# ruppelb/Large-Scale-ViT-SLAM

Hardware: AMD Instinct MI355X
Metric: chunks/sec (16-frame 518x518) + ViT MFMA util% (higher is better)
Workload: dtype bf16; 1 GPU; VGGT aggregator forward (DINOv2-L/14-reg + 24x frame/global AA blocks), 1 chunk of 16 frames 518x518, layers 4/11/17/23 emitted; frames=16, parallelism=replicas x1

## Files before the change

### include/vggt_mi355x.h

```cpp
#ifndef VGGT_MI355X_H
#define VGGT_MI355X_H

#include <stddef.h>
#include <stdint.h>

#ifdef __cplusplus
extern "C" {
#endif

#define VGGT_OK 0
#define VGGT_ERR_SHAPE (-1)
#define VGGT_ERR_ALIGN (-2)
#define VGGT_ERR_HIP (-3)
#define VGGT_ERR_UNSUPPORTED (-4)

#define VGGT_DTYPE_F32 0
#define VGGT_DTYPE_BF16 1

#define VGGT_EPI_BF16 0
#define VGGT_EPI_GELU_BF16 1
#define VGGT_EPI_RESID_F32 2
#define VGGT_EPI_F32 3

#define VGGT_ROPE_NONE 0
#define VGGT_ROPE_2D 1
#define VGGT_ROPE_1D 2

const char* vggt_version(void);

#define VGGT_TUNE_GEMM_TILE 1
#define VGGT_TUNE_ATTN_WAVES 2
#define VGGT_TUNE_ATTN_VARIANT 3
#define VGGT_TUNE_CONV_PF2 4
#define VGGT_TUNE_ATTN16 5
#define VGGT_TUNE_LINEAR_ONE_LAUNCH 6
#define VGGT_TUNE_LINEAR_SPLIT_K 7
#define VGGT_TUNE_LINEAR_WK 8
#define VGGT_TUNE_GEMM_BALANCE 10
#define VGGT_TUNE_ATTN_TAIL_SPLIT 11
int vggt_tune(int knob, int value);

#define VGGT_STREAM_SHORT_WORKGROUPS 1
int vggt_set_stream_config(void* stream, int cus, int flags);

int vggt_gemm_bf16(const void* A, int64_t lda, const void* W, int64_t ldw, const float* bias, int M, int N, int K,
                   int epi, void* out, int64_t ldo, const float* gamma, float* out2, int64_t ldo2, void* stream);

int vggt_gemm_bf16_gelu_pre(const void* A, int64_t lda, const void* W, int64_t ldw, const float* bias, int M, int N,
                            int K, void* out, int64_t ldo, void* pre, int64_t ldp, void* stream);

int vggt_gemm_qkv(const void* A, int64_t lda, const void* W, int64_t ldw, const float* bias, int M, int H, int D, int K,
                  void* out, int64_t ldo, const float* qw, const float* qb, const float* kw, const float* kb, float eps,
                  int rope_mode, const int32_t* pos, int period, const float* cos_tab, const float* sin_tab,
                  int tab_len, void* stream);

int vggt_gemm_headnorm(const void* A, int64_t lda, const void* W, int64_t ldw, const float* bias, int M, int N, int H,
                       int D, int K, void* out, int64_t ldo, const float* nw, const float* nb, float eps, int rope_mode,
                       const int32_t* pos, int period, const float* cos_tab, const float* sin_tab, int tab_len,
                       void* stream);

#define VGGT_GEMM_ENTRY_BF16 0
#define VGGT_GEMM_ENTRY_GELU_PRE 1
#define VGGT_GEMM_ENTRY_QKV 2
#define VGGT_GEMM_ENTRY_HEADNORM 3
#define VGGT_GEMM_FAMILY_128 0
#define VGGT_GEMM_FAMILY_RING 1
#define VGGT_GEMM_FAMILY_TWO 2
#define VGGT_GEMM_FAMILY_PP 3
#define VGGT_GEMM_FAMILY_PPP 4
typedef struct {
  int family;
  int bm, bn;
  int epi;
  int fk;
  int grid, lds;
  int sched;
  int split_rows;
  int rc;
  int dev_cus;
} vggt_gemm_form_t;
int vggt_gemm_form(int entry, int epi, int has_out2, int M, int N, int K, int H, int D, int rope_mode, int period,
                   int tab_len, int64_t lda, int64_t ldw, int64_t ldo, int64_t ldo2, int stream_cus, int stream_flags,
                   int force, vggt_gemm_form_t* form);

int vggt_layernorm(const void* x, int in_dtype, int64_t ldx, const float* w, const float* b, float eps, int M, int C,
                   void* y, int out_dtype, int64_t ldy, void* stream);

int vggt_resid_add_layernorm(float* x, int64_t ldx, const void* y, int64_t ldy, const float* gamma, float* out2,
                             int64_t ldo2, const float* w, const float* b, float eps, int M, int C, void* xn,
                             int64_t ldn, void* stream);

int vggt_resid_add_layernorm_nostore(const float* x, int64_t ldx, const void* y, int64_t ldy, const float* gamma,
                                     const float* w, const float* b, float eps, int M, int C, void* xn, int64_t ldn,
                                     void* stream);
int vggt_resid_add2_layernorm(float* x, int64_t ldx, const void* y, int64_t ldy, const float* gamma, const void* y2,
                              int64_t ldy2, const float* gamma2, float* out2, int64_t ldo2, const float* w,
                              const float* b, float eps, int M, int C, void* xn, int64_t ldn, void* stream);

int vggt_headnorm_rope(void* buf, int64_t ld, int col_off, int M, int H, int D, const float* w, const float* b,
                       float eps, int rope_mode, const int32_t* pos, int period, const float* cos_tab,
                       const float* sin_tab, int tab_len, void* stream);

int vggt_qknorm_rope(void* qkv, int64_t ld, int M, int H, int D, const float* qw, const float* qb, const float* kw,
                     const float* kb, float eps, int rope_mode, const int32_t* pos, int period, const float* cos_tab,
                     const float* sin_tab, int tab_len, void* stream);

int vggt_qknorm_rope_out(const void* src, int64_t lds, void* dst, int64_t ldd, int M, int H, int D, const float* qw,
                         const float* qb, const float* kw, const float* kb, float eps, int rope_mode,
                         const int32_t* pos, int period, const float* cos_tab, const float* sin_tab, int tab_len,
                         void* stream);
int vggt_headnorm_rope_out(const void* src, int64_t lds, void* dst, int64_t ldd, int M, int H, int D, const float* w,
                           const float* b, float eps, int rope_mode, const int32_t* pos, int period,
                           const float* cos_tab, const float* sin_tab, int tab_len, void* stream);

int vggt_attention_fwd(const void* q, int64_t ldq, int64_t q_bstride, const void* k, int64_t ldk, int64_t k_bstride,
                       const void* v, int64_t ldv, int64_t v_bstride, void* o, int64_t ldo, int64_t o_bstride,
                       int batch, int heads, int nq, int nk, int D, float scale, void* stream);

int vggt_attention_fwd_ws(const void* q, int64_t ldq, int64_t q_bstride, const void* k, int64_t ldk,
                          int64_t k_bstride, const void* v, int64_t ldv, int64_t v_bstride, void* o, int64_t ldo,
                          int64_t o_bstride, int batch, int heads, int nq, int nk, int D, float scale, void* ws,
                          size_t ws_bytes, void* stream);
// ... 187 lines not shown
```

### large-scale-vit-slam_amd/aligned_vggt/_native.py

```python
from __future__ import annotations

import ctypes
import os
from typing import Optional

import torch

from .runtime import Workspace, scratch_table

_PKG_ROOT = os.path.dirname(os.path.dirname(os.path.abspath(__file__)))
LIB_PATH = os.environ.get("VGGT_MI355X_LIB", os.path.join(_PKG_ROOT, "lib", "libvggt_mi355x.so"))
HEADER_PATH = os.path.join(os.path.dirname(_PKG_ROOT), "include", "vggt_mi355x.h")

VGGT_OK, VGGT_ERR_SHAPE, VGGT_ERR_ALIGN, VGGT_ERR_HIP, VGGT_ERR_UNSUPPORTED = 0, -1, -2, -3, -4
DTYPE_F32, DTYPE_BF16 = 0, 1
EPI_BF16, EPI_GELU_BF16, EPI_RESID_F32, EPI_F32 = 0, 1, 2, 3
ROPE_NONE, ROPE_2D, ROPE_1D = 0, 1, 2

_ERR = {VGGT_ERR_SHAPE: "unsupported or inconsistent shape", VGGT_ERR_ALIGN: "misaligned pointer or leading dimension",
        VGGT_ERR_HIP: "HIP launch/runtime error", VGGT_ERR_UNSUPPORTED: "unsupported mode or dtype"}

_vp, _i, _i64, _f = ctypes.c_void_p, ctypes.c_int, ctypes.c_int64, ctypes.c_float
_SIGS = {
    "vggt_tune": [_i, _i],
# ... 52 lines not shown
    "vggt_upsample_bilinear_f32": [_vp, _i, _i, _i, _i, _vp, _i, _i, _vp, _vp],
    "vggt_dpt_activate": [_vp, _i64, _i64, _i, _i, _i, _vp, _vp, _vp, _vp],
    "vggt_irls_sim3": [_vp, _i64, _vp, _i64, _vp, _i64, _vp, _i64, _i, _i64, _f, _f, _i, _f, _vp, _vp, _vp, _vp,
                       ctypes.c_size_t, _vp],
    "vggt_sim3_points": [_vp, _i64, _i, _i64, _vp, _vp, _vp, _i64, _vp],
    "vggt_scale_f32": [_vp, _i64, _i, _i64, _vp, _vp],
    "vggt_pose_compose": [_vp, _vp, _vp, _vp, _i, _vp, _i, _i, _i, _i, _i, _vp, _vp, _vp],
    "vggt_attention_fwd_lse": [_vp, _i64, _i64, _vp, _i64, _i64, _vp, _i64, _i64, _vp, _i64, _i64, _vp, _i, _i, _i,
                               _i, _i, _f, _vp],
    "vggt_attention_bwd": [_vp, _i64, _i64, _vp, _i64, _i64, _vp, _i64, _vp, _vp, _i64, _i64, _vp, _vp, _vp, _i64,
                           _vp, _vp, _i64, _i, _i, _i, _i, _i, _f, _vp],
    "vggt_attention_small_bwd": [_vp, _i64, _i64, _vp, _i64, _i64, _vp, _i64, _vp, _i64, _i64, _vp, _i64, _i64, _vp,
                                 _vp, _i64, _i64, _i, _i, _i, _i, _i, _i, _f, _vp],
    "vggt_layernorm_bwd": [_vp, _i, _i64, _vp, _f, _vp, _i, _i64, _vp, _i, _i64, _i, _i, _i, _i, _i, _i, _i, _i, _vp,
                           _vp, _vp, ctypes.c_size_t, _vp],
    "vggt_headnorm_rope_bwd": [_vp, _i64, _vp, _i64, _i, _i, _i, _i, _i, _vp, _vp, _f, _i, _vp, _i, _vp, _vp, _i, _vp,
                               _vp, _vp, _vp, _vp, ctypes.c_size_t, _vp],
    "vggt_colsum": [_vp, _i, _i64, _i, _i, _vp, _i, _vp, ctypes.c_size_t, _vp],
    "vggt_layerscale_bwd": [_vp, _i64, _vp, _i, _i64, _vp, _vp, _i, _i64, _i, _i, _vp, _vp, _vp, ctypes.c_size_t,
                            _vp],
    "vggt_gelu_fwd": [_vp, _i, _i64, _vp, _i, _i64, _i, _i, _vp],
    "vggt_gelu_bwd": [_vp, _i, _i64, _vp, _i, _i64, _vp, _i, _i64, _i, _i, _vp, _vp, ctypes.c_size_t, _vp],
    "vggt_resid_scale_add": [_vp, _i64, _vp, _i, _i64, _vp, _i, _i, _vp],
    "vggt_gemm_bf16_gelu_pre": [_vp, _i64, _vp, _i64, _vp, _i, _i, _i, _vp, _i64, _vp, _i64, _vp],
    "vggt_resid_scale_add_from": [_vp, _i64, _vp, _i64, _vp, _i, _i64, _vp, _i, _i, _vp],
    "vggt_qknorm_rope_out": [_vp, _i64, _vp, _i64, _i, _i, _i, _vp, _vp, _vp, _vp, _f, _i, _vp, _i, _vp, _vp, _i, _vp],
    "vggt_headnorm_rope_out": [_vp, _i64, _vp, _i64, _i, _i, _i, _vp, _vp, _f, _i, _vp, _i, _vp, _vp, _i, _vp],
    "vggt_transpose_b16": [_vp, _i64, _i, _i, _vp, _i64, _i, _vp],
    "vggt_wgrad_f32": [_vp, _i64, _vp, _i64, _i, _i, _i, _vp, _i64, _i, _vp],
    "vggt_wgrad_bias_f32": [_vp, _i64, _vp, _i64, _i, _i, _i, _vp, _i64, _vp, _i, _vp],
    "vggt_wgrad_bf16": [_vp, _i64, _vp, _i64, _i, _i, _i, _vp, _i64, _i, _vp, ctypes.c_size_t, _vp],
    "vggt_batch_dot_f32": [_vp, _vp, _i64, _i, _i64, _vp, _vp, ctypes.c_size_t, _vp],
    "vggt_nn1": [_vp, _i64, _vp, _vp, _i64, _vp, _i, _i64, _i64, _i, _vp, _vp, _i, _vp, ctypes.c_size_t, _vp],
    "vggt_nn1_plan": [_i, _i64, _i64, _i],
    "vggt_nn1_pair_stats": [_vp, _i64, _vp, _vp, _i64, _vp, _vp, _i, _i64, _i64, _vp, _vp, ctypes.c_size_t, _vp],
}
_WS_FNS = {"vggt_colred_workspace_bytes": [_i, _i], "vggt_layernorm_bwd_workspace_bytes": [_i, _i],
           "vggt_headnorm_rope_bwd_workspace_bytes": [_i, _i], "vggt_batch_dot_workspace_bytes": [_i, _i64],
           "vggt_wgrad_bf16_workspace_bytes": [_i, _i, _i], "vggt_attention_ws_bytes": [_i, _i, _i, _i, _i, _vp],
           "vggt_nn1_workspace_bytes": [_i, _i64, _i64]}

_lib = None

EVENT_HOOK = None


def lib() -> ctypes.CDLL:
    global _lib
    if _lib is None:
        if not os.path.exists(LIB_PATH):
            raise RuntimeError(f"libvggt_mi355x.so not found at {LIB_PATH}: build it with "
                               f"`make -C large-scale-vit-slam_amd/csrc` (or __graft_entry__.build()); "
                               f"there is no CPU fallback for the HIP hot path")
        L = ctypes.CDLL(LIB_PATH)
        for name, argt in _SIGS.items():
            fn = getattr(L, name)
            fn.argtypes = argt
            fn.restype = ctypes.c_int
        L.vggt_version.restype = ctypes.c_char_p
        L.vggt_irls_workspace_bytes.argtypes = [_i]
        L.vggt_irls_workspace_bytes.restype = ctypes.c_size_t
        for name, argt in _WS_FNS.items():
            fn = getattr(L, name)
            fn.argtypes = argt
            fn.restype = ctypes.c_size_t
        _lib = L
    return _lib


def version() -> str:
    return lib().vggt_version().decode()


TUNE_GEMM_TILE = 1
TUNE_ATTN_WAVES = 2
TUNE_ATTN_VARIANT = 3
TUNE_CONV_PF2 = 4
TUNE_ATTN16 = 5
TUNE_LINEAR_ONE_LAUNCH = 6
TUNE_LINEAR_SPLIT_K = 7
TUNE_LINEAR_WK = 8
TUNE_GEMM_BALANCE = 10
TUNE_ATTN_TAIL_SPLIT = 11


def tune(knob: int, value: int) -> int:
    rc = lib().vggt_tune(knob, value)
    if rc == VGGT_ERR_UNSUPPORTED:
        raise ValueError(f"vggt_tune: unsupported knob/value ({knob}, {value})")
    return rc


STREAM_SHORT_WORKGROUPS = 1


def set_stream_config(stream: int, cus: int, flags: int = 0) -> int:
    rc = lib().vggt_set_stream_config(ctypes.c_void_p(stream), cus, flags)
    if rc < 0:
        raise ValueError(f"vggt_set_stream_config: rejected ({rc})")
    return rc


def mfma_probe(iters: int = 200_000, random: bool = True, seconds: float = 2.0, device=None) -> dict:
    import statistics
    device = torch.device(device or "cuda")
    ncu = torch.cuda.get_device_properties(device).multi_processor_count
    g = torch.Generator(device="cpu").manual_seed(0)
    n = ncu * 256 * 16
    ops = (torch.randn(n, generator=g) if random else torch.zeros(n)).to(torch.bfloat16).to(device)
    stamps = torch.zeros(ncu * 4, dtype=torch.int64, device=device)
    sink = torch.empty(ncu * 256, dtype=torch.float32, device=device)
    st = ctypes.c_void_p(torch.cuda.current_stream(device).cuda_stream)
    launch = lambda: _check(lib().vggt_mfma_probe(_p(stamps), _p(sink), _p(ops), ncu, iters, st),
                            "vggt_mfma_probe")
    import time
    t_end = time.perf_counter() + seconds
    while time.perf_counter() < t_end:
        launch()
        torch.cuda.synchronize(device)
    a = torch.cuda.Event(enable_timing=True)
    b = torch.cuda.Event(enable_timing=True)
    a.record()
    launch()
    b.record()
    b.synchronize()
    ms = a.elapsed_time(b)
    sp = stamps.view(ncu, 4).cpu().tolist()
    clocks = [(t1 - t0) / (r1 - r0) * 100e6 for t0, t1, r0, r1 in sp if r1 > r0]
    clk = statistics.median(clocks)
    flop = ncu * 4 * iters * 8 * 32768.0
    return {"tflops": round(flop / (ms * 1e-3) / 1e12, 1), "clock_ghz": round(clk / 1e9, 3),
            "flop_per_cycle_per_cu": round(flop / ncu / (ms * 1e-3 * clk), 1), "ms": round(ms, 3), "cus": ncu,
            "operands": "random bf16" if random else "zeros"}


def _check(rc: int, name: str) -> None:
    if rc != VGGT_OK:
        raise RuntimeError(f"{name}: {_ERR.get(rc, 'error')} (code {rc})")


def _dev(t: torch.Tensor, name: str) -> None:
    if t.device.type != "cuda":
        raise RuntimeError(f"{name}: tensor on {t.device}; the MI355X hot path runs on HIP devices only")


def _p(t: Optional[torch.Tensor]):
    return None if t is None else ctypes.c_void_p(t.data_ptr())


def _stream() -> ctypes.c_void_p:
    return ctypes.c_void_p(torch.cuda.current_stream().cuda_stream)


def _ld(t: torch.Tensor) -> int:
    if t.dim() != 2 or t.stride(1) != 1:
        raise RuntimeError("expected a 2-D row-major (unit inner stride) view")
    return t.stride(0)


def gemm_bf16(a: torch.Tensor, w: torch.Tensor, bias: torch.Tensor, out: torch.Tensor, epi: int,
              gamma: Optional[torch.Tensor] = None, out2: Optional[torch.Tensor] = None) -> torch.Tensor:
    _dev(a, "gemm_bf16")
    M, K = a.shape
    N = w.shape[0]
    assert a.dtype == torch.bfloat16 and w.dtype == torch.bfloat16 and w.shape[1] == K
    assert out.shape[0] == M and out.shape[1] == N
# ... 813 lines not shown
```

### large-scale-vit-slam_amd/csrc/attention.hip

```cpp
#include <math.h>
#include <string.h>

#include <algorithm>
#include <mutex>
#include <type_traits>
#include <vector>

#include "common.h"
#include "tune.h"

namespace {

typedef __attribute__((ext_vector_type(4))) short s16x4;
typedef __attribute__((ext_vector_type(8))) short s16x8;
typedef int int32x4 __attribute__((ext_vector_type(4)));

constexpr int BKV = 64;
constexpr float THR = 8.0f;

struct AttnArgs {
  const bf16_t* q;
  const bf16_t* k;
  const bf16_t* v;
  bf16_t* o;
  int64_t ldq, ldk, ldv, ldo;
  int64_t qbs, kbs, vbs, obs;
  int batch, heads, nq, nk;
  float c;
  float* lse;
  int n_full, parts, part_tiles;
  float* ws;
};

constexpr int SPLIT_BQ = 256;
constexpr int SPLIT_SLAB = SPLIT_BQ * 64 + 2 * SPLIT_BQ;

__device__ __forceinline__ void dma16(int32x4 rsrc, uint32_t voff, uint32_t lds) {
  uint32_t keep;
  asm volatile("s_mov_b32 %0, m0\n\ts_mov_b32 m0, %3\n\ts_nop 0\n\tbuffer_load_dwordx4 %1, %2, 0 offen lds\n\t"
               "s_mov_b32 m0, %0"
               : "=&s"(keep)
               : "v"(voff), "s"(rsrc), "s"(lds)
               : "memory");
}

__device__ __forceinline__ int32x4 make_rsrc(const void* base, uint32_t nbytes) {
  const uint64_t b = (uint64_t)base;
  int32x4 r;
  r[0] = __builtin_amdgcn_readfirstlane((uint32_t)b);
  r[1] = __builtin_amdgcn_readfirstlane((uint32_t)(b >> 32)) & 0xffff;
  r[2] = __builtin_amdgcn_readfirstlane(nbytes);
  r[3] = 0x00020000;
  return r;
}

template <int D>
__device__ __forceinline__ int k_swz(int row, int chunk) {
  if constexpr (D == 64) return chunk ^ ((row >> 1) & 7);
  else return chunk ^ (row & 15);
}
template <int D>
__device__ __forceinline__ int v_swz(int row, int chunk) {
  if constexpr (D == 64) return chunk ^ (((row >> 1) & 1) << 2);
  else return chunk ^ ((row & 3) << 2);
}

constexpr int V_HOIST_K = 1;
constexpr int V_MAX4 = 2;
constexpr int V_SUM4 = 4;
constexpr int V_MFMA_SUM = 8;
constexpr int V_PIPE_QK = 16;
constexpr int V_OFFSET_FREE = 32;
constexpr int V_EXACT = 64;
constexpr int V_SPLIT_TILE = 256;
constexpr int V_DMA_AHEAD = 512;
constexpr int V_STAMPS = 1024;
constexpr int V_DMA_HALF = 2048;
constexpr int V_NO_PRIO = 4096;
constexpr int V_KEY_SPLIT = 8192;
constexpr int ID_FORM16 = 128;
constexpr int V_33 = V_OFFSET_FREE | V_HOIST_K;
constexpr int V_96 = V_OFFSET_FREE | V_EXACT;
constexpr int V_161 = V_33 | ID_FORM16;
constexpr int V_289 = V_33 | V_SPLIT_TILE;
constexpr int V_545 = V_33 | V_DMA_AHEAD;
constexpr int V_2081 = V_33 | V_DMA_HALF;
constexpr int V_4129 = V_33 | V_NO_PRIO;
constexpr int V_19 = V_PIPE_QK | V_MAX4 | V_HOIST_K;
constexpr int V_23 = V_19 | V_SUM4;
constexpr int V_LEGACY = V_HOIST_K | V_MAX4 | V_SUM4 | V_MFMA_SUM;
constexpr int STAMP_N = 8;
template <int D, int NW, int VAR>
__global__ __launch_bounds__(NW * 64, 8 / NW) void attn_fwd_kernel(AttnArgs a) {
  constexpr int BQ = NW * 32;
  constexpr int ROWB = D * 2;
  constexpr int TILEB = BKV * ROWB;
  constexpr int NKS = D / 16;
  constexpr int NDB = D / 32;
  constexpr int RPI = 1024 / ROWB;
  constexpr int CPR = ROWB / 16;
  constexpr int IPW = TILEB / 1024 / NW;
  constexpr int NSLOT = (VAR & (V_PIPE_QK | V_DMA_AHEAD)) ? 3 : 2;
  __shared__ __attribute__((aligned(16))) char smem[NSLOT * 2 * TILEB];

  const int lane = threadIdx.x & 63;
  const int wave = __builtin_amdgcn_readfirstlane(threadIdx.x >> 6);
  const int hl = lane >> 5;
  if constexpr (NW == 8 && !(VAR & V_NO_PRIO)) {
    if (wave >= 4) __builtin_amdgcn_s_setprio(1);
  }
  const int nqb = (a.nq + BQ - 1) / BQ;
  constexpr bool SPLIT = (VAR & V_KEY_SPLIT) != 0;
  int bid, nk = a.nk, key0 = 0, slab = -1;
  if constexpr (SPLIT) {
    const int bx = blockIdx.x;
    if (bx < a.n_full) {
      bid = xcd_remap(bx, a.n_full);
    } else {
      slab = xcd_remap(bx - a.n_full, (int)gridDim.x - a.n_full);
      const int part = slab % a.parts;
      bid = a.n_full + slab / a.parts;
      key0 = part * a.part_tiles * BKV;
      nk = part == a.parts - 1 ? a.nk - key0 : a.part_tiles * BKV;
    }
  } else {
    bid = xcd_remap(blockIdx.x, nqb * a.heads * a.batch);
  }
  const int qb = bid % nqb;
  const int bh = bid / nqb;
  const int h = bh % a.heads;
  const int b = bh / a.heads;

  const bf16_t* qp = a.q + (int64_t)b * a.qbs * a.ldq + h * D;
  const bf16_t* kp = a.k + ((int64_t)b * a.kbs + key0) * a.ldk + h * D;
  const bf16_t* vp = a.v + ((int64_t)b * a.vbs + key0) * a.ldv + h * D;

  const int qrow = qb * BQ + wave * 32 + (lane & 31);
  const int qr = min(qrow, a.nq - 1);
  bf16x8 qf[NKS];
#pragma unroll
  for (int ks = 0; ks < NKS; ++ks) qf[ks] = *(const bf16x8*)(qp + (int64_t)qr * a.ldq + ks * 16 + 8 * hl);
  if constexpr ((VAR & V_OFFSET_FREE) && !(VAR & V_EXACT)) {
#pragma unroll
    for (int ks = 0; ks < NKS; ++ks)
#pragma unroll
      for (int j = 0; j < 8; ++j) qf[ks][j] = (__bf16)((float)qf[ks][j] * a.c);
  }
#pragma unroll
  for (int ks = 0; ks < NKS; ++ks) asm volatile("" : "+v"(qf[ks]));

  constexpr bool DMAH = (VAR & V_DMA_HALF) && NW == 8;
  constexpr int IPWX = DMAH ? 2 * IPW : IPW;
  const int pbase = DMAH ? (wave >= 4 ? wave - 4 : 0) * IPWX : wave * IPW;
  uint32_t koff[IPWX], voff[IPWX];
#pragma unroll
  for (int i = 0; i < IPWX; ++i) {
    const int row = (pbase + i) * RPI + lane / CPR;
    const int cp = lane % CPR;
    koff[i] = (uint32_t)(row * a.ldk + k_swz<D>(row, cp) * 8) * 2u;
    voff[i] = (uint32_t)(row * a.ldv + v_swz<D>(row, cp) * 8) * 2u;
  }
  const uint32_t lds0 = __builtin_amdgcn_readfirstlane((uint32_t)(uintptr_t)LDS_PTR(smem)) + pbase * 1024;
  const int kstep = BKV * (int)a.ldk * 2, vstep = BKV * (int)a.ldv * 2;
  const int kbytes = nk * (int)a.ldk * 2, vbytes = nk * (int)a.ldv * 2;

  auto stage = [&](int buf, int t) {
    const int ko = kstep * t, vo = vstep * t;
    const int32x4 kr = make_rsrc((const char*)kp + ko, (uint32_t)max(kbytes - ko, 0));
    const int32x4 vr = make_rsrc((const char*)vp + vo, (uint32_t)max(vbytes - vo, 0));
    const uint32_t d = lds0 + buf * 2 * TILEB;
    if (!DMAH || wave >= 4) {
#pragma unroll
      for (int i = 0; i < IPWX; ++i) {
        dma16(kr, koff[i], d + i * 1024);
        dma16(vr, voff[i], d + TILEB + i * 1024);
      }
    }
  };

  uint32_t ka[NKS];
  {
    const int key = lane & 31;
#pragma unroll
    for (int ks = 0; ks < NKS; ++ks) ka[ks] = key * ROWB + (k_swz<D>(key, 2 * ks + hl) << 4);
  }
  uint32_t va[NDB];
  {
    const int g = (lane >> 4) & 1, qq = (lane >> 2) & 3, pp = lane & 3;
    const int r0 = 4 * hl + qq;
#pragma unroll
    for (int db = 0; db < NDB; ++db) {
      const int col = db * 32 + 16 * g + 4 * pp;
      va[db] = TILEB + r0 * ROWB + (v_swz<D>(r0, col >> 3) << 4) + (col & 7) * 2;
    }
  }

  f32x16 o[NDB];
#pragma unroll
  for (int i = 0; i < NDB; ++i) o[i] = f32x16{};
  constexpr float M_UNSET = -1e30f;
  float m_run = (VAR & V_OFFSET_FREE) ? M_UNSET : -INFINITY, l_run = 0.f;
  float lb_run = 0.f;
  f32x16 lsum = f32x16{};
  float lim = THR, limv = 256.0f;
// ... 619 lines not shown
    __syncthreads();
    for (int t = 0; t < nt; t += 2) {
      if (t + 1 < nt) stage(1, t + 1);
      body(I0{}, t);
      asm volatile("s_waitcnt vmcnt(0)" ::: "memory");
      __syncthreads();
      if (t + 1 >= nt) break;
      if (t + 2 < nt) stage(0, t + 2);
      body(I1{}, t + 1);
      asm volatile("s_waitcnt vmcnt(0)" ::: "memory");
      __syncthreads();
    }
  };
  auto reset = [&]() {
#pragma unroll
    for (int db = 0; db < 4; ++db)
#pragma unroll
      for (int qb = 0; qb < 2; ++qb) o[db][qb] = f32x4{};
    l[0] = l[1] = 0.f;
  };
  auto allsum = [](float x) {
    const auto s16 = __builtin_amdgcn_permlane16_swap(__float_as_uint(x), __float_as_uint(x), false, false);
    x = __uint_as_float(s16[0]) + __uint_as_float(s16[1]);
    const auto s32 = __builtin_amdgcn_permlane32_swap(__float_as_uint(x), __float_as_uint(x), false, false);
    return __uint_as_float(s32[0]) + __uint_as_float(s32[1]);
  };
  auto allmax = [](float x) {
    const auto s16 = __builtin_amdgcn_permlane16_swap(__float_as_uint(x), __float_as_uint(x), false, false);
    x = fmaxf(__uint_as_float(s16[0]), __uint_as_float(s16[1]));
    const auto s32 = __builtin_amdgcn_permlane32_swap(__float_as_uint(x), __float_as_uint(x), false, false);
    return fmaxf(__uint_as_float(s32[0]), __uint_as_float(s32[1]));
  };

  if (threadIdx.x == 0) redo = 0;
  reset();
  sweep([&](auto bufc, int t) { soft_pv(bufc, t, std::false_type{}); });
  l[0] = allsum(l[0]);
  l[1] = allsum(l[1]);
  const bool bad = !(l[0] >= 0x1p-60f && l[0] <= 0x1p100f) || !(l[1] >= 0x1p-60f && l[1] <= 0x1p100f);
  if (__builtin_amdgcn_ballot_w64(bad) != 0 && lane == 0) redo = 1;
  __syncthreads();
  if (redo) {
    float mx[2] = {-INFINITY, -INFINITY};
    sweep([&](auto bufc, int t) {
      const S8 s = scores(bufc, t);
#pragma unroll
      for (int qb = 0; qb < 2; ++qb)
#pragma unroll
        for (int kb = 0; kb < 4; ++kb)
          mx[qb] = fmaxf(fmaxf(mx[qb], fmaxf(s.v[kb][qb][0], s.v[kb][qb][1])), fmaxf(s.v[kb][qb][2], s.v[kb][qb][3]));
    });
    m[0] = allmax(mx[0]);
    m[1] = allmax(mx[1]);
    reset();
    sweep([&](auto bufc, int t) { soft_pv(bufc, t, std::true_type{}); });
    l[0] = allsum(l[0]);
    l[1] = allsum(l[1]);
  }

#pragma unroll
  for (int qb = 0; qb < 2; ++qb) {
    const int qrow = q0 + 16 * qb;
    const float inv = 1.f / l[qb];
    if (a.lse && g == 0 && qrow < a.nq) a.lse[((int64_t)b * a.heads + h) * a.nq + qrow] = m[qb] + __log2f(l[qb]);
    if (qrow < a.nq) {
      bf16_t* op = a.o + ((int64_t)b * a.obs + qrow) * a.ldo + h * D;
#pragma unroll
      for (int db = 0; db < 4; ++db) {
        uint2 pk;
        pk.x = pack_bf2(o[db][qb][0] * inv, o[db][qb][1] * inv);
        pk.y = pack_bf2(o[db][qb][2] * inv, o[db][qb][3] * inv);
        *(uint2*)(op + db * 16 + 4 * g) = pk;
      }
    }
  }
}

__global__ __launch_bounds__(256) void attn_split_merge_kernel(AttnArgs a, int n_tail) {
  constexpr int D = 64;
  const int tid = blockIdx.x * 256 + threadIdx.x;
  const int lane = tid & 63, c = (tid >> 6) & 7, wave = (tid >> 9) & 7, tu = tid >> 12;
  if (tu >= n_tail) return;
  const int nqb = (a.nq + SPLIT_BQ - 1) / SPLIT_BQ;
  const int bid = a.n_full + tu;
  const int qb = bid % nqb, bh = bid / nqb;
  const int h = bh % a.heads, b = bh / a.heads;
  const int r = wave * 32 + (lane & 31), hl = lane >> 5;
  const int qrow = qb * SPLIT_BQ + r;
  if (qrow >= a.nq) return;
  const float* sp = a.ws + (int64_t)tu * a.parts * SPLIT_SLAB;
  float mx = -INFINITY;
  for (int p = 0; p < a.parts; ++p) mx = fmaxf(mx, sp[(int64_t)p * SPLIT_SLAB + SPLIT_BQ * D + r * 2]);
  f32x4 num = f32x4{0.f, 0.f, 0.f, 0.f};
  float den = 0.f;
  for (int p = 0; p < a.parts; ++p) {
    const float* pp = sp + (int64_t)p * SPLIT_SLAB;
    const f32x2 ml = *(const f32x2*)(pp + SPLIT_BQ * D + r * 2);
    const float w = __builtin_amdgcn_exp2f(ml[0] - mx);
    num += w * *(const f32x4*)(pp + ((wave * 8 + c) * 64 + lane) * 4);
    den += w * ml[1];
  }
  const float inv = 1.f / den;
  uint2 pk;
  pk.x = pack_bf2(num[0] * inv, num[1] * inv);
  pk.y = pack_bf2(num[2] * inv, num[3] * inv);
  bf16_t* op = a.o + ((int64_t)b * a.obs + qrow) * a.ldo + h * D;
  *(uint2*)(op + (c >> 2) * 32 + 8 * (c & 3) + 4 * hl) = pk;
}

inline int attn_cu_count(hipStream_t s) {
  static int dev_cus = [] {
    int dev = 0, n = 0;
    if (hipGetDevice(&dev) != hipSuccess ||
        hipDeviceGetAttribute(&n, hipDeviceAttributeMultiprocessorCount, dev) != hipSuccess || n <= 0)
      n = 256;
    return n;
  }();
  const int n = vggt_stream_cu_count(s);
  return n > 0 ? n : dev_cus;
}

constexpr double PLAN_UNIT_OVH = 2.0;
constexpr double PLAN_TILE_US = 1.87, PLAN_BYTES_PER_US = 3.5e6, PLAN_MERGE_US = 5.0;
constexpr double PLAN_MIN_GAIN = 0.03;
constexpr int PLAN_MIN_PART_TILES = 86;

struct PlanSeg {
  int count;
  double len;
};
double plan_makespan(int cus, const PlanSeg* segs, int nseg) {
  std::vector<double> rem((size_t)cus * 2, 0.0);
  std::vector<int> cnt((size_t)cus, 0);
  int seg = 0, left = nseg > 0 ? segs[0].count : 0, resident = 0;
  double now = 0.0;
  auto more = [&]() {
    while (seg < nseg && left == 0) {
      ++seg;
      if (seg < nseg) left = segs[seg].count;
    }
    return seg < nseg;
  };
  for (;;) {
    for (int want = 0; want < 2; ++want)
      for (int cu = 0; cu < cus; ++cu)
        if (cnt[cu] == want && more()) {
          rem[cu * 2 + cnt[cu]] = segs[seg].len;
          ++cnt[cu];
          --left;
          ++resident;
        }
    if (resident == 0) return now;
    double dt = 1e300;
    for (int cu = 0; cu < cus; ++cu)
      for (int i = 0; i < cnt[cu]; ++i) dt = std::min(dt, rem[cu * 2 + i] * cnt[cu] * 0.5);
    now += dt;
    for (int cu = 0; cu < cus; ++cu) {
      const int n = cnt[cu];
      const double done = dt * 2.0 / (n > 0 ? n : 1);
      int keep = 0;
      for (int i = 0; i < n; ++i) {
        const double r = rem[cu * 2 + i] - done;
        if (r > 1e-9) rem[cu * 2 + keep++] = r;
        else --resident;
      }
      cnt[cu] = keep;
    }
  }
}

inline void split_shape(int nt, int want, int* parts, int* part_tiles) {
  const int p = std::max(1, std::min(want, nt));
  *part_tiles = (nt + p - 1) / p;
  *parts = (nt + *part_tiles - 1) / *part_tiles;
}

}

extern "C" int vggt_attention_split_plan(int batch, int heads, int nq, int nk, int D, int cus, int* tail_blocks,
                                         int* parts) {
  if (tail_blocks) *tail_blocks = 0;
  if (parts) *parts = 0;
  if (batch <= 0 || heads <= 0 || nq < 4096 || nk <= 0 || D != 64 || cus <= 0) return 0;
  const int64_t units64 = (int64_t)((nq + SPLIT_BQ - 1) / SPLIT_BQ) * heads * batch;
  const int slots = 2 * cus, nt = (nk + BKV - 1) / BKV;
  if (units64 < slots || units64 > (1 << 24) || units64 % slots == 0 || nt < 2) return 0;
  const int units = (int)units64, tail = units % slots;
  struct Entry {
    int key[4], tail, parts;
  };
  static std::mutex mu;
  static std::vector<Entry> cache;
  const int key[4] = {units, nq, nk, cus};
  std::lock_guard<std::mutex> lk(mu);
  const Entry* hit = nullptr;
  for (const Entry& e : cache)
    if (!memcmp(e.key, key, sizeof key)) hit = &e;
  if (!hit) {
    const PlanSeg whole[1] = {{units, nt + PLAN_UNIT_OVH}};
    const double t0 = plan_makespan(cus, whole, 1);
    double best = t0;
    int best_p = 0;
    for (int want = 2; want <= 4; ++want) {
      int p, pt;
      split_shape(nt, want, &p, &pt);
      if (p != want || pt < PLAN_MIN_PART_TILES) continue;
      const PlanSeg segs[3] = {{units - tail, nt + PLAN_UNIT_OVH},
                               {tail * (p - 1), pt + PLAN_UNIT_OVH},
                               {tail, nt - (p - 1) * pt + PLAN_UNIT_OVH}};
      const double bytes = 2.0 * tail * p * SPLIT_SLAB * 4.0;
      const double t = plan_makespan(cus, segs, 3) + (bytes / PLAN_BYTES_PER_US + PLAN_MERGE_US) / PLAN_TILE_US;
      if (t < best) best = t, best_p = want;
    }
    if (cache.size() >= 64) cache.clear();
    cache.push_back(Entry{{units, nq, nk, cus}, tail, (t0 - best) >= PLAN_MIN_GAIN * t0 ? best_p : 0});
    hit = &cache.back();
  }
  if (hit->parts < 2) return 0;
  if (tail_blocks) *tail_blocks = hit->tail;
  if (parts) *parts = hit->parts;
  return 1;
}

namespace {
void tail_split_of(int batch, int heads, int nq, int nk, int cus, int* tail, int* parts, int* part_tiles) {
  *tail = *parts = *part_tiles = 0;
  const int knob = g_vggt_attn_tail_split;
  const int64_t units = (int64_t)((nq + SPLIT_BQ - 1) / SPLIT_BQ) * heads * batch;
  const int nt = (nk + BKV - 1) / BKV;
  int t = 0, p = 0;
  if (knob < 0 || units > (1 << 18)) return;
  if (knob > 0) {
    p = knob & 0xff;
    t = (int)std::min<int64_t>(knob >> 8, units);
  } else if (!vggt_attention_split_plan(batch, heads, nq, nk, 64, cus, &t, &p)) {
    return;
  }
  int pr, pt;
  split_shape(nt, std::min(p, 4), &pr, &pt);
  if (pr < 2 || t <= 0) return;
  *tail = t;
  *parts = pr;
  *part_tiles = pt;
}

struct AttnForm {
  bool form16;
  int nw, var;
  bool key_split;
};

AttnForm attn_resolve(int variant, int waves, int attn16, int dma_half, int D, int nq) {
  const bool two_ok = (variant & V_OFFSET_FREE) && (variant & (V_EXACT | V_HOIST_K)) == V_HOIST_K;
  const int nw = (waves == 8 && nq >= 4096) ? 8 : (waves == 2 && two_ok) ? 2 : 4;
  const bool d64 = D == 64, wide = d64 && nw != 2;
  if (wide && (variant == V_161 || (variant == V_33 && (attn16 == 1 || (attn16 == 2 && nw == 4)))))
    return {true, nw, 0, false};
  if (d64 && (variant == V_19 || variant == V_23)) return {false, nw, variant, false};
  if (d64 && nw == 8 && variant == V_33 && dma_half) return {false, 8, V_2081, true};
  if (wide && (variant == V_2081 || variant == V_4129)) return {false, nw, nw == 8 ? variant : V_33, false};
  if (wide && (variant == V_545 || variant == V_289)) return {false, nw, variant, false};
  if (variant & V_OFFSET_FREE) return {false, nw, variant & (V_OFFSET_FREE | V_EXACT | V_HOIST_K), false};
  return {false, nw, variant & V_LEGACY, false};
}

AttnForm attn_resolve_now(int D, int nq) {
  return attn_resolve(g_vggt_attn_variant, g_vggt_attn_waves, g_vggt_attn16, g_vggt_attn_dma_half, D, nq);
}

#define VGGT_ATTN_D_NW(X, V) X(64, 4, V) X(64, 8, V) X(128, 4, V) X(128, 8, V)
#define VGGT_ATTN_KERNELS(X)                                                                              \
  VGGT_ATTN_D_NW(X, V_HOIST_K | V_MAX4) VGGT_ATTN_D_NW(X, V_HOIST_K | V_MAX4 | V_SUM4)                    \
  VGGT_ATTN_D_NW(X, V_HOIST_K | V_MAX4 | V_MFMA_SUM) VGGT_ATTN_D_NW(X, V_LEGACY)                          \
  VGGT_ATTN_D_NW(X, V_OFFSET_FREE) VGGT_ATTN_D_NW(X, V_33)                                                \
  VGGT_ATTN_D_NW(X, V_96) VGGT_ATTN_D_NW(X, V_96 | V_HOIST_K)                                             \
  X(64, 2, V_33) X(128, 2, V_33)                                                                          \
  X(64, 4, V_19) X(64, 8, V_19) X(64, 4, V_23) X(64, 8, V_23)                                             \
  X(64, 4, V_289) X(64, 8, V_289) X(64, 4, V_545) X(64, 8, V_545)                                         \
  X(64, 8, V_2081) X(64, 8, V_2081 | V_KEY_SPLIT) X(64, 8, V_4129)                                        \
  X(64, 4, V_33 | V_STAMPS) X(64, 8, V_33 | V_STAMPS) X(64, 8, V_2081 | V_STAMPS) X(64, 8, V_4129 | V_STAMPS)

bool attn_has(const AttnForm& f, int D) {
  if (f.form16) return D == 64 && (f.nw == 4 || f.nw == 8);
#define VGGT_ATTN_IS(DD, NWW, V) \
  if (D == DD && f.nw == NWW && f.var == (V)) return true;
  VGGT_ATTN_KERNELS(VGGT_ATTN_IS)
#undef VGGT_ATTN_IS
  return false;
}

int attn_launch(const AttnForm& f, int D, const AttnArgs& a, int grid, hipStream_t s) {
  if (!attn_has(f, D)) return VGGT_ERR_UNSUPPORTED;
  if (f.form16) {
    if (f.nw == 8) attn16_fwd_kernel<8><<<grid, 512, 0, s>>>(a);
    else attn16_fwd_kernel<4><<<grid, 256, 0, s>>>(a);
  }
#define VGGT_ATTN_TRY(DD, NWW, V) \
  else if (D == DD && f.nw == NWW && f.var == (V)) attn_fwd_kernel<DD, NWW, (V)><<<grid, NWW * 64, 0, s>>>(a);
  VGGT_ATTN_KERNELS(VGGT_ATTN_TRY)
#undef VGGT_ATTN_TRY
  HIP_LAUNCH_CHECK();
  return VGGT_OK;
}

AttnForm attn_resolve_stamps(int variant, int waves, int dma_half, int nq) {
  const int v = (variant == V_2081 || variant == V_4129) ? variant : V_33;
  AttnForm f = attn_resolve(v, waves == 2 ? 4 : waves, 0, variant == V_33 && dma_half, 64, nq);
  f.var |= V_STAMPS;
  return f;
}

int attn_args(AttnArgs* a, const void* q, int64_t ldq, int64_t q_bstride, const void* k, int64_t ldk,
              int64_t k_bstride, const void* v, int64_t ldv, int64_t v_bstride, void* o, int64_t ldo, int64_t o_bstride,
              int batch, int heads, int nq, int nk, int D, float scale, float* lse) {
  if (batch <= 0 || heads <= 0 || nq <= 0 || nk <= 0) return VGGT_ERR_SHAPE;
  if (D != 64 && D != 128) return VGGT_ERR_UNSUPPORTED;
  if ((ldq | ldk | ldv | ldo) % 8 || ((uintptr_t)q | (uintptr_t)k | (uintptr_t)v | (uintptr_t)o) % 16)
    return VGGT_ERR_ALIGN;
  if ((uint64_t)nk * (uint64_t)(ldk > ldv ? ldk : ldv) * 2 >= (1ull << 31)) return VGGT_ERR_SHAPE;
  *a = AttnArgs{(const bf16_t*)q, (const bf16_t*)k, (const bf16_t*)v, (bf16_t*)o, ldq, ldk, ldv, ldo,
                q_bstride, k_bstride, v_bstride, o_bstride, batch, heads, nq, nk,
                scale * 1.4426950408889634f, lse};
  return VGGT_OK;
}

int attn_grid(int nw, int batch, int heads, int nq) { return ((nq + nw * 32 - 1) / (nw * 32)) * heads * batch; }
}

extern "C" int vggt_attention_fwd_form(int D, int nq, int* form16, int* waves, int* var) {
  const AttnForm f = attn_resolve_now(D, nq);
  if (form16) *form16 = f.form16;
  if (waves) *waves = f.nw;
  if (var) *var = f.var;
  if (D != 64 && D != 128) return VGGT_ERR_UNSUPPORTED;
  return attn_has(f, D) ? VGGT_OK : VGGT_ERR_UNSUPPORTED;
}

extern "C" int vggt_attention_stamps_form(int nq, int* waves, int* var) {
  const AttnForm f = attn_resolve_stamps(g_vggt_attn_variant, g_vggt_attn_waves, g_vggt_attn_dma_half, nq);
  if (waves) *waves = f.nw;
  if (var) *var = f.var;
  return attn_has(f, 64) ? VGGT_OK : VGGT_ERR_UNSUPPORTED;
}

extern "C" size_t vggt_attention_ws_bytes(int batch, int heads, int nq, int nk, int D, void* stream) {
  if (batch <= 0 || heads <= 0 || nq <= 0 || nk <= 0 || !attn_resolve_now(D, nq).key_split) return 0;
  int tail, parts, pt;
  tail_split_of(batch, heads, nq, nk, attn_cu_count((hipStream_t)stream), &tail, &parts, &pt);
  return (size_t)tail * parts * SPLIT_SLAB * sizeof(float);
}

extern "C" int vggt_attention_fwd_ws(const void* q, int64_t ldq, int64_t q_bstride, const void* k, int64_t ldk,
                                     int64_t k_bstride, const void* v, int64_t ldv, int64_t v_bstride, void* o,
                                     int64_t ldo, int64_t o_bstride, int batch, int heads, int nq, int nk, int D,
                                     float scale, void* ws, size_t ws_bytes, void* stream) {
  if (ws && (uintptr_t)ws % 16) return VGGT_ERR_ALIGN;
  AttnArgs a;
  const int rc = attn_args(&a, q, ldq, q_bstride, k, ldk, k_bstride, v, ldv, v_bstride, o, ldo, o_bstride, batch, heads,
                           nq, nk, D, scale, nullptr);
  if (rc != VGGT_OK) return rc;
  hipStream_t s = (hipStream_t)stream;
  AttnForm f = attn_resolve_now(D, nq);
  const int nwg = attn_grid(f.nw, batch, heads, nq);
  int tail = 0, parts = 0, pt = 0;
  if (f.key_split && ws) tail_split_of(batch, heads, nq, nk, attn_cu_count(s), &tail, &parts, &pt);
  if (parts < 2) return attn_launch(f, D, a, nwg, s);
  if (ws_bytes < (size_t)tail * parts * SPLIT_SLAB * sizeof(float)) return VGGT_ERR_SHAPE;
  a.n_full = nwg - tail;
  a.parts = parts;
  a.part_tiles = pt;
  a.ws = (float*)ws;
  f.var |= V_KEY_SPLIT;
  const int rc2 = attn_launch(f, D, a, a.n_full + tail * parts, s);
  if (rc2 != VGGT_OK) return rc2;
  attn_split_merge_kernel<<<tail * 16, 256, 0, s>>>(a, tail);
  HIP_LAUNCH_CHECK();
  return VGGT_OK;
}

extern "C" int vggt_attention_fwd(const void* q, int64_t ldq, int64_t q_bstride, const void* k, int64_t ldk,
                                  int64_t k_bstride, const void* v, int64_t ldv, int64_t v_bstride, void* o,
                                  int64_t ldo, int64_t o_bstride, int batch, int heads, int nq, int nk, int D,
                                  float scale, void* stream) {
  return vggt_attention_fwd_ws(q, ldq, q_bstride, k, ldk, k_bstride, v, ldv, v_bstride, o, ldo, o_bstride, batch,
                               heads, nq, nk, D, scale, nullptr, 0, stream);
}

extern "C" int vggt_attention_stamps(const void* q, int64_t ldq, int64_t q_bstride, const void* k, int64_t ldk,
                                     int64_t k_bstride, const void* v, int64_t ldv, int64_t v_bstride, void* o,
                                     int64_t ldo, int64_t o_bstride, unsigned long long* stamps, int batch, int heads,
                                     int nq, int nk, float scale, void* stream) {
  if (!stamps) return VGGT_ERR_SHAPE;
  AttnArgs a;
  const int rc = attn_args(&a, q, ldq, q_bstride, k, ldk, k_bstride, v, ldv, v_bstride, o, ldo, o_bstride, batch, heads,
                           nq, nk, 64, scale, (float*)(void*)stamps);
  if (rc != VGGT_OK) return rc;
  const AttnForm f = attn_resolve_stamps(g_vggt_attn_variant, g_vggt_attn_waves, g_vggt_attn_dma_half, nq);
  return attn_launch(f, 64, a, attn_grid(f.nw, batch, heads, nq), (hipStream_t)stream);
}

extern "C" int vggt_attention_fwd_lse(const void* q, int64_t ldq, int64_t q_bstride, const void* k, int64_t ldk,
                                      int64_t k_bstride, const void* v, int64_t ldv, int64_t v_bstride, void* o,
                                      int64_t ldo, int64_t o_bstride, float* lse, int batch, int heads, int nq, int nk,
                                      int D, float scale, void* stream) {
  if (!lse) return VGGT_ERR_SHAPE;
  AttnArgs a;
  const int rc = attn_args(&a, q, ldq, q_bstride, k, ldk, k_bstride, v, ldv, v_bstride, o, ldo, o_bstride, batch, heads,
                           nq, nk, D, scale, lse);
  if (rc != VGGT_OK) return rc;
  return attn_launch(AttnForm{false, 4, V_96, false}, D, a, attn_grid(4, batch, heads, nq), (hipStream_t)stream);
}
```

### large-scale-vit-slam_amd/csrc/capi.cpp

```cpp
#include "../../include/vggt_mi355x.h"

extern "C" const char* vggt_version(void) { return "vggt_mi355x 0.1 gfx950"; }

#include <stdlib.h>

#include <atomic>
#include <initializer_list>
#include <mutex>

#include "tune.h"

namespace {
int env_or(const char* name, int dflt) {
  const char* e = getenv(name);
  return e ? atoi(e) : dflt;
}
bool attn_variant_ok(int v) {
  for (int ok : {3, 7, 11, 15, 19, 23, 32, 33, 96, 97, 161, 289, 545, 2081, 4129})
    if (v == ok) return true;
  return false;
}
int attn_variant_env() {
  const int v = env_or("VGGT_ATTN_VARIANT", 33);
  return attn_variant_ok(v) ? v : 33;
}
}

int g_vggt_gemm_tile = env_or("VGGT_GEMM", -1);
int g_vggt_attn_waves = env_or("VGGT_ATTN_WAVES", 8);
int g_vggt_attn_variant = attn_variant_env();
int g_vggt_attn_dma_half = env_or("VGGT_ATTN_DMA_HALF", 1) != 0;
int g_vggt_attn16 = env_or("VGGT_ATTN16", 2);
int g_vggt_conv_pf2 = env_or("VGGT_CONV_PF2", 1);
int g_vggt_linear_one_launch = env_or("VGGT_LINEAR_ONE_LAUNCH", 1);
int g_vggt_linear_split_k = env_or("VGGT_LINEAR_SPLIT_K", 128);
int g_vggt_linear_wk = env_or("VGGT_LINEAR_WK", 64);
int g_vggt_gemm_balance = env_or("VGGT_GEMM_BALANCE", 0);
const GemmKnobs g_vggt_gemm_knobs = {env_or("VGGT_GEMM_MID", 0),   env_or("VGGT_GEMM_PERSIST", 7),
                                     env_or("VGGT_GEMM_BM", 0),    env_or("VGGT_GEMM_FULLK", 5),
                                     env_or("VGGT_GEMM_GM", 4) & 255, env_or("VGGT_GEMM_SPLITDMA", 1) != 0,
                                     env_or("VGGT_HEADNORM_TILE", -1)};
int g_vggt_attn_tail_split = env_or("VGGT_ATTN_TAIL_SPLIT", -1);

extern "C" int vggt_tune(int knob, int value) {
  int prev;
  switch (knob) {
    case VGGT_TUNE_GEMM_TILE:
      if (value < -1 || value > 9) return VGGT_ERR_UNSUPPORTED;
      prev = g_vggt_gemm_tile;
      g_vggt_gemm_tile = value;
      return prev;
    case VGGT_TUNE_ATTN_WAVES:
      if (value != 2 && value != 4 && value != 8) return VGGT_ERR_UNSUPPORTED;
      prev = g_vggt_attn_waves;
      g_vggt_attn_waves = value;
      return prev;
    case VGGT_TUNE_ATTN_VARIANT:
      if (!attn_variant_ok(value)) return VGGT_ERR_UNSUPPORTED;
      prev = g_vggt_attn_variant;
      g_vggt_attn_variant = value;
      return prev;
    case VGGT_TUNE_ATTN16:
      if (value < 0 || value > 2) return VGGT_ERR_UNSUPPORTED;
      prev = g_vggt_attn16;
      g_vggt_attn16 = value;
      return prev;
    case VGGT_TUNE_LINEAR_ONE_LAUNCH:
      if (value != 0 && value != 1) return VGGT_ERR_UNSUPPORTED;
      prev = g_vggt_linear_one_launch;
      g_vggt_linear_one_launch = value;
      return prev;
    case VGGT_TUNE_LINEAR_SPLIT_K:
      if (value < 16 || value > 4096 || (value & (value - 1))) return VGGT_ERR_UNSUPPORTED;
      prev = g_vggt_linear_split_k;
      g_vggt_linear_split_k = value;
      return prev;
    case VGGT_TUNE_LINEAR_WK:
      if (value != 0 && (value < 64 || value > 4096 || (value & (value - 1)))) return VGGT_ERR_UNSUPPORTED;
      prev = g_vggt_linear_wk;
      g_vggt_linear_wk = value;
      return prev;
    case VGGT_TUNE_GEMM_BALANCE:
      if (value != 0 && value != 1) return VGGT_ERR_UNSUPPORTED;
      prev = g_vggt_gemm_balance;
      g_vggt_gemm_balance = value;
      return prev;
    case VGGT_TUNE_ATTN_TAIL_SPLIT:
      if (value < -1 || (value > 0 && ((value & 0xff) < 2 || (value >> 8) < 1))) return VGGT_ERR_UNSUPPORTED;
      prev = g_vggt_attn_tail_split;
      g_vggt_attn_tail_split = value;
      return prev;
    case VGGT_TUNE_CONV_PF2:
      if (value != 0 && value != 1) return VGGT_ERR_UNSUPPORTED;
      prev = g_vggt_conv_pf2;
      g_vggt_conv_pf2 = value;
      return prev;
    default: return VGGT_ERR_UNSUPPORTED;
  }
}

namespace {
constexpr int kMaxStreams = 16;
std::atomic<void*> g_cfg_stream[kMaxStreams];
std::atomic<int> g_cfg_cus[kMaxStreams];
std::atomic<int> g_cfg_flags[kMaxStreams];
std::mutex g_cfg_mu;
int find_cfg(void* stream) {
  if (!stream) return -1;
  for (int i = 0; i < kMaxStreams; ++i)
    if (g_cfg_stream[i].load(std::memory_order_acquire) == stream) return i;
  return -1;
}
}

int vggt_stream_cu_count(void* stream) {
  const int i = find_cfg(stream);
  return i < 0 ? 0 : g_cfg_cus[i].load(std::memory_order_relaxed);
}

int vggt_stream_flags(void* stream) {
  const int i = find_cfg(stream);
  return i < 0 ? 0 : g_cfg_flags[i].load(std::memory_order_relaxed);
}

extern "C" int vggt_set_stream_config(void* stream, int cus, int flags) {
  if (!stream || cus < 0 || (flags & ~VGGT_STREAM_SHORT_WORKGROUPS)) return VGGT_ERR_SHAPE;
  std::lock_guard<std::mutex> lk(g_cfg_mu);
  int slot = find_cfg(stream);
  const int prev = slot < 0 ? 0 : (g_cfg_cus[slot].load(std::memory_order_relaxed) |
                                    g_cfg_flags[slot].load(std::memory_order_relaxed) << 16);
  if (cus == 0 && flags == 0) {
    if (slot >= 0) g_cfg_stream[slot].store(nullptr, std::memory_order_release);
    return prev;
  }
  if (slot < 0) {
    for (int i = 0; i < kMaxStreams && slot < 0; ++i)
      if (!g_cfg_stream[i].load(std::memory_order_relaxed)) slot = i;
    if (slot < 0) return VGGT_ERR_UNSUPPORTED;
    g_cfg_cus[slot].store(cus, std::memory_order_relaxed);
    g_cfg_flags[slot].store(flags, std::memory_order_relaxed);
    g_cfg_stream[slot].store(stream, std::memory_order_release);
  } else {
    g_cfg_cus[slot].store(cus, std::memory_order_relaxed);
    g_cfg_flags[slot].store(flags, std::memory_order_relaxed);
  }
  return prev;
}
```

Baseline: 10.80 chunks/s.

## Plan attention tail key-split per batch element and enable it by default

Reworks the attention tail-split plan so the ragged tail of query blocks is computed per batch element (a periodic mapping of block ids) instead of once over the whole batch. The plan now uses the device CU count and ignores any per-stream CU setting. The default knob changes from disabled (-1) to auto (0), so key-split tail attention with a merge kernel now runs by default. This targets wave-quantization idle time in the global attention tail, at the cost of workspace, an extra merge launch, and the split-key overhead.

```diff
diff --git a/include/vggt_mi355x.h b/include/vggt_mi355x.h
--- a/include/vggt_mi355x.h
+++ b/include/vggt_mi355x.h
@@ -38,6 +38,7 @@
 #define VGGT_TUNE_LINEAR_WK 8
 #define VGGT_TUNE_GEMM_BALANCE 10
 #define VGGT_TUNE_ATTN_TAIL_SPLIT 11
+#define VGGT_ATTN_TAIL_SPLIT_PER_ELEMENT (1 << 30)
 int vggt_tune(int knob, int value);
 
 #define VGGT_STREAM_SHORT_WORKGROUPS 1
diff --git a/large-scale-vit-slam_amd/aligned_vggt/_native.py b/large-scale-vit-slam_amd/aligned_vggt/_native.py
--- a/large-scale-vit-slam_amd/aligned_vggt/_native.py
+++ b/large-scale-vit-slam_amd/aligned_vggt/_native.py
@@ -158,6 +158,7 @@
 TUNE_LINEAR_WK = 8
 TUNE_GEMM_BALANCE = 10
 TUNE_ATTN_TAIL_SPLIT = 11
+ATTN_TAIL_SPLIT_PER_ELEMENT = 1 << 30
 
 
 def tune(knob: int, value: int) -> int:
diff --git a/large-scale-vit-slam_amd/csrc/attention.hip b/large-scale-vit-slam_amd/csrc/attention.hip
--- a/large-scale-vit-slam_amd/csrc/attention.hip
+++ b/large-scale-vit-slam_amd/csrc/attention.hip
@@ -30,6 +30,7 @@
   float* lse;
   int n_full, parts, part_tiles;
   float* ws;
+  int unit_period, full_pp;
 };
 
 constexpr int SPLIT_BQ = 256;
@@ -115,11 +116,12 @@
   if constexpr (SPLIT) {
     const int bx = blockIdx.x;
     if (bx < a.n_full) {
-      bid = xcd_remap(bx, a.n_full);
+      const int w = xcd_remap(bx, a.n_full);
+      bid = w / a.full_pp * a.unit_period + w % a.full_pp;
     } else {
       slab = xcd_remap(bx - a.n_full, (int)gridDim.x - a.n_full);
-      const int part = slab % a.parts;
-      bid = a.n_full + slab / a.parts;
+      const int part = slab % a.parts, tu = slab / a.parts, tail_pp = a.unit_period - a.full_pp;
+      bid = tu / tail_pp * a.unit_period + a.full_pp + tu % tail_pp;
       key0 = part * a.part_tiles * BKV;
       nk = part == a.parts - 1 ? a.nk - key0 : a.part_tiles * BKV;
     }
@@ -905,7 +907,8 @@
   const int lane = tid & 63, c = (tid >> 6) & 7, wave = (tid >> 9) & 7, tu = tid >> 12;
   if (tu >= n_tail) return;
   const int nqb = (a.nq + SPLIT_BQ - 1) / SPLIT_BQ;
-  const int bid = a.n_full + tu;
+  const int tail_pp = a.unit_period - a.full_pp;
+  const int bid = tu / tail_pp * a.unit_period + a.full_pp + tu % tail_pp;
   const int qb = bid % nqb, bh = bid / nqb;
   const int h = bh % a.heads, b = bh / a.heads;
   const int r = wave * 32 + (lane & 31), hl = lane >> 5;
@@ -931,7 +934,7 @@
   *(uint2*)(op + (c >> 2) * 32 + 8 * (c & 3) + 4 * hl) = pk;
 }
 
-inline int attn_cu_count(hipStream_t s) {
+inline int attn_cu_count() {
   static int dev_cus = [] {
     int dev = 0, n = 0;
     if (hipGetDevice(&dev) != hipSuccess ||
@@ -939,8 +942,7 @@
       n = 256;
     return n;
   }();
-  const int n = vggt_stream_cu_count(s);
-  return n > 0 ? n : dev_cus;
+  return dev_cus;
 }
 
 constexpr double PLAN_UNIT_OVH = 2.0;
@@ -1005,7 +1007,7 @@
   if (tail_blocks) *tail_blocks = 0;
   if (parts) *parts = 0;
   if (batch <= 0 || heads <= 0 || nq < 4096 || nk <= 0 || D != 64 || cus <= 0) return 0;
-  const int64_t units64 = (int64_t)((nq + SPLIT_BQ - 1) / SPLIT_BQ) * heads * batch;
+  const int64_t units64 = (int64_t)((nq + SPLIT_BQ - 1) / SPLIT_BQ) * heads;
   const int slots = 2 * cus, nt = (nk + BKV - 1) / BKV;
   if (units64 < slots || units64 > (1 << 24) || units64 % slots == 0 || nt < 2) return 0;
   const int units = (int)units64, tail = units % slots;
@@ -1046,25 +1048,34 @@
 }
 
 namespace {
-void tail_split_of(int batch, int heads, int nq, int nk, int cus, int* tail, int* parts, int* part_tiles) {
-  *tail = *parts = *part_tiles = 0;
+struct TailSplit {
+  int period, periods, tail, parts, part_tiles;
+  size_t ws_bytes() const { return (size_t)periods * tail * parts * SPLIT_SLAB * sizeof(float); }
+};
+TailSplit tail_split_of(int batch, int heads, int nq, int nk) {
+  TailSplit ts = {0, 0, 0, 0, 0};
   const int knob = g_vggt_attn_tail_split;
-  const int64_t units = (int64_t)((nq + SPLIT_BQ - 1) / SPLIT_BQ) * heads * batch;
+  const int64_t per_elem = (int64_t)((nq + SPLIT_BQ - 1) / SPLIT_BQ) * heads, units = per_elem * batch;
   const int nt = (nk + BKV - 1) / BKV;
   int t = 0, p = 0;
-  if (knob < 0 || units > (1 << 18)) return;
+  if (knob < 0 || units > (1 << 18)) return ts;
+  bool global = false;
   if (knob > 0) {
     p = knob & 0xff;
-    t = (int)std::min<int64_t>(knob >> 8, units);
-  } else if (!vggt_attention_split_plan(batch, heads, nq, nk, 64, cus, &t, &p)) {
-    return;
+    global = !(knob & VGGT_ATTN_TAIL_SPLIT_PER_ELEMENT);
+    t = (int)std::min<int64_t>((knob & ~VGGT_ATTN_TAIL_SPLIT_PER_ELEMENT) >> 8, global ? units : per_elem);
+  } else if (!vggt_attention_split_plan(1, heads, nq, nk, 64, attn_cu_count(), &t, &p)) {
+    return ts;
   }
   int pr, pt;
   split_shape(nt, std::min(p, 4), &pr, &pt);
-  if (pr < 2 || t <= 0) return;
-  *tail = t;
-  *parts = pr;
-  *part_tiles = pt;
+  if (pr < 2 || t <= 0) return ts;
+  ts.period = (int)(global ? units : per_elem);
+  ts.periods = global ? 1 : batch;
+  ts.tail = t;
+  ts.parts = pr;
+  ts.part_tiles = pt;
+  return ts;
 }
 
 struct AttnForm {
@@ -1168,9 +1179,8 @@
 
 extern "C" size_t vggt_attention_ws_bytes(int batch, int heads, int nq, int nk, int D, void* stream) {
   if (batch <= 0 || heads <= 0 || nq <= 0 || nk <= 0 || !attn_resolve_now(D, nq).key_split) return 0;
-  int tail, parts, pt;
-  tail_split_of(batch, heads, nq, nk, attn_cu_count((hipStream_t)stream), &tail, &parts, &pt);
-  return (size_t)tail * parts * SPLIT_SLAB * sizeof(float);
+  (void)stream;
+  return tail_split_of(batch, heads, nq, nk).ws_bytes();
 }
 
 extern "C" int vggt_attention_fwd_ws(const void* q, int64_t ldq, int64_t q_bstride, const void* k, int64_t ldk,
@@ -1185,16 +1195,19 @@
   hipStream_t s = (hipStream_t)stream;
   AttnForm f = attn_resolve_now(D, nq);
   const int nwg = attn_grid(f.nw, batch, heads, nq);
-  int tail = 0, parts = 0, pt = 0;
-  if (f.key_split && ws) tail_split_of(batch, heads, nq, nk, attn_cu_count(s), &tail, &parts, &pt);
-  if (parts < 2) return attn_launch(f, D, a, nwg, s);
-  if (ws_bytes < (size_t)tail * parts * SPLIT_SLAB * sizeof(float)) return VGGT_ERR_SHAPE;
+  TailSplit ts = {0, 0, 0, 0, 0};
+  if (f.key_split && ws) ts = tail_split_of(batch, heads, nq, nk);
+  if (ts.parts < 2) return attn_launch(f, D, a, nwg, s);
+  if (ws_bytes < ts.ws_bytes()) return VGGT_ERR_SHAPE;
+  const int tail = ts.periods * ts.tail;
   a.n_full = nwg - tail;
-  a.parts = parts;
-  a.part_tiles = pt;
+  a.parts = ts.parts;
+  a.part_tiles = ts.part_tiles;
   a.ws = (float*)ws;
+  a.unit_period = ts.period;
+  a.full_pp = ts.period - ts.tail;
   f.var |= V_KEY_SPLIT;
-  const int rc2 = attn_launch(f, D, a, a.n_full + tail * parts, s);
+  const int rc2 = attn_launch(f, D, a, a.n_full + tail * ts.parts, s);
   if (rc2 != VGGT_OK) return rc2;
   attn_split_merge_kernel<<<tail * 16, 256, 0, s>>>(a, tail);
   HIP_LAUNCH_CHECK();
diff --git a/large-scale-vit-slam_amd/csrc/capi.cpp b/large-scale-vit-slam_amd/csrc/capi.cpp
--- a/large-scale-vit-slam_amd/csrc/capi.cpp
+++ b/large-scale-vit-slam_amd/csrc/capi.cpp
@@ -40,7 +40,7 @@
                                      env_or("VGGT_GEMM_BM", 0),    env_or("VGGT_GEMM_FULLK", 5),
                                      env_or("VGGT_GEMM_GM", 4) & 255, env_or("VGGT_GEMM_SPLITDMA", 1) != 0,
                                      env_or("VGGT_HEADNORM_TILE", -1)};
-int g_vggt_attn_tail_split = env_or("VGGT_ATTN_TAIL_SPLIT", -1);
+int g_vggt_attn_tail_split = env_or("VGGT_ATTN_TAIL_SPLIT", 0);
 
 extern "C" int vggt_tune(int knob, int value) {
   int prev;
@@ -86,7 +86,9 @@
       g_vggt_gemm_balance = value;
       return prev;
     case VGGT_TUNE_ATTN_TAIL_SPLIT:
-      if (value < -1 || (value > 0 && ((value & 0xff) < 2 || (value >> 8) < 1))) return VGGT_ERR_UNSUPPORTED;
+      if (value < -1 || value == VGGT_ATTN_TAIL_SPLIT_PER_ELEMENT ||
+          (value > 0 && ((value & 0xff) < 2 || ((value & ~VGGT_ATTN_TAIL_SPLIT_PER_ELEMENT) >> 8) < 1)))
+        return VGGT_ERR_UNSUPPORTED;
       prev = g_vggt_attn_tail_split;
       g_vggt_attn_tail_split = value;
       return prev;
```

Result: faster. 10.92 chunks/s (median of 6 runs) (+1.1%).
